# meyerls/PEGASUS

Hardware: AMD Instinct MI355X
Metric: rendered views/sec (RGB+depth+mask) on 2M-Gaussian scene @800x800 (higher is better)
Workload: dtype f32

## Files before the change

### pegasus_amd/csrc/tilebin.hip.h

```cpp
#pragma once
#include <type_traits>

#include "composite.hip.h"
#include "cull.hip.h"
#include "pgr_common.h"

namespace pgr {

constexpr int BIN_CHUNK = 4096;
#ifndef PGR_BIN_THREADS
#define PGR_BIN_THREADS 512
#endif
constexpr int BIN_THREADS = PGR_BIN_THREADS;
constexpr int BIN_LDS_TILES = 16384;

__device__ __forceinline__ uint2 pack_rect(int minx, int miny, int maxx, int maxy) {
    return make_uint2((uint32_t)minx | ((uint32_t)miny << 16), (uint32_t)maxx | ((uint32_t)maxy << 16));
}

struct BinView {
    const uint2* rects;
    const float4* splats;
    uint32_t* tile_count;
    uint32_t* rel;
    uint2* ranges;
    uint32_t* counters;
    uint2* bucket;
    uint32_t* gauss_sorted;
    uint64_t* alt;
    uint32_t* obj_last;
    int32_t n_env;
    const int32_t* tie_index;
    const uint32_t* tie_inv;
    uint2* records;
};


template <int CTRL, int ROW_MASK = 0xF, bool BOUND_CTRL = true>
__device__ __forceinline__ uint32_t dpp_u32(uint32_t v) {
    return (uint32_t)__builtin_amdgcn_update_dpp(0, (int)v, CTRL, ROW_MASK, 0xF, BOUND_CTRL);
}

__device__ __forceinline__ uint32_t wave_inclusive_scan(uint32_t v) {
    v += dpp_u32<0x111>(v);
    v += dpp_u32<0x112>(v);
    v += dpp_u32<0x114>(v);
    v += dpp_u32<0x118>(v);
    v += dpp_u32<0x142, 0xA, false>(v);
    v += dpp_u32<0x143, 0xC, false>(v);
    return v;
}

__device__ __forceinline__ uint32_t wave_inclusive_max(uint32_t v) {
    v = max(v, dpp_u32<0x111>(v));
    v = max(v, dpp_u32<0x112>(v));
    v = max(v, dpp_u32<0x114>(v));
    v = max(v, dpp_u32<0x118>(v));
    v = max(v, dpp_u32<0x142, 0xA, false>(v));
    v = max(v, dpp_u32<0x143, 0xC, false>(v));
    return v;
}

constexpr int BIN_STAGE_WORDS = WAVE * 12 + WAVE;
constexpr int BIN_THREADS_SMALL = 1024;
__host__ __device__ inline size_t bin_lds_bytes(int tiles, int threads) {
    return ((size_t)(tiles < BIN_LDS_TILES ? tiles : BIN_LDS_TILES) + 3) / 4 * 16 + (size_t)(threads / WAVE) * BIN_STAGE_WORDS * 4 + 16;
}

struct BinLayers {
    const int32_t* layer_id;
    int32_t layer_tiles;
    int32_t layer_rows;
    int32_t n_layers;
};
constexpr uint32_t VERDICT_WINDOWS = 62;
constexpr uint32_t VERDICT_REGION_WORDS = 192;

template <bool SCATTER, int THREADS>
__global__ __launch_bounds__(THREADS) void bin_kernel(const BinView* __restrict__ views, int n, int grid_x,
                                                          int tiles, int W, int H, const uint32_t* __restrict__ vis,
                                                          int vis_words, int verdict_groups,
                                                          BinLayers layers = BinLayers{nullptr, 0, 0, 0}) {
    extern __shared__ __attribute__((aligned(16))) uint32_t lds[];
    constexpr int BIN_WAVES = THREADS / WAVE;
    const BinView& bv = views[blockIdx.y];
    if (SCATTER && gload(bv.counters + 1)) return;
    const int chunk = blockIdx.x;
    const int begin = chunk * BIN_CHUNK, end = min(n, begin + BIN_CHUNK);
    const int lane = threadIdx.x & (WAVE - 1), wave = threadIdx.x / WAVE;
    const bool layered = layers.layer_id != nullptr;
    const int hist_words = (min(layered ? layers.layer_tiles : tiles, BIN_LDS_TILES) + 3) / 4 * 4;
    float4* const stage = reinterpret_cast<float4*>(lds + hist_words + wave * BIN_STAGE_WORDS);
    uint32_t* const heads = reinterpret_cast<uint32_t*>(stage + WAVE * 3);
    uint32_t* const ctrl = lds + hist_words + BIN_WAVES * BIN_STAGE_WORDS;
    constexpr int GROUPS = BIN_CHUNK / WAVE;
    static_assert(GROUPS == WAVE, "one visibility bit per lane of a wave");
    int pass_first = 0, pass_last = (tiles - 1) / BIN_LDS_TILES;
    if (layered) {
        if (begin >= end) return;
        pass_first = max(1, min(layers.n_layers + 1, (int)gload(layers.layer_id + begin)));
        pass_last = min(layers.n_layers, (int)gload(layers.layer_id + end - 1));
    }
    for (int lp = pass_first; lp <= pass_last; ++lp) {
        const int lo = layered ? (lp - 1) * layers.layer_tiles : lp * BIN_LDS_TILES;
        const int span = layered ? layers.layer_tiles : min(BIN_LDS_TILES, tiles - lo);
        const int row_off = layered ? (lp - 1) * layers.layer_rows : 0;
        for (int t = threadIdx.x; t < span; t += THREADS)
            lds[t] = SCATTER ? gload(bv.ranges + lo + t).x + gload(bv.rel + (size_t)chunk * tiles + lo + t) : 0u;
        if (wave == 0) {
            const int b = begin + lane * WAVE;
            bool visible = b < end;
            if (visible && vis) visible = (vis[(size_t)(b / WAVE) * vis_words + (blockIdx.y >> 5)] >> (blockIdx.y & 31)) & 1u;
            const uint64_t m = __ballot(visible);
            if (lane == 0) { ctrl[0] = 0u; ctrl[1] = (uint32_t)m; ctrl[2] = (uint32_t)(m >> 32); }
        }
        __syncthreads();
        const uint64_t vis_bits = ((uint64_t)ctrl[2] << 32) | ctrl[1];
        auto take_ticket = [&]() {
            for (;;) {
                uint32_t ticket = 0;
                if (lane == 0) ticket = atomicAdd(&ctrl[0], 1u);
                ticket = (uint32_t)__builtin_amdgcn_readfirstlane((int)ticket);
                if (ticket >= (uint32_t)GROUPS || ((vis_bits >> ticket) & 1ull)) return ticket;
            }
        };
        for (uint32_t ticket = take_ticket(); ticket < (uint32_t)GROUPS; ticket = take_ticket()) {
            const int base = begin + (int)ticket * WAVE;
            bool has_region = base / WAVE < verdict_groups;
            if (layered) {
                const int l0 = gload(layers.layer_id + base), l1 = gload(layers.layer_id + min(base + WAVE, end) - 1);
                if (lp < l0 || lp > l1) continue;
                has_region = has_region && l0 == l1;
            }
            uint32_t* const region = reinterpret_cast<uint32_t*>(bv.records) + (size_t)(base / WAVE) * VERDICT_REGION_WORDS;
            uint64_t* const ballots = reinterpret_cast<uint64_t*>(region + WAVE);
            const int i = base + lane;
            const int ic = i < end ? i : end - 1;
            uint2 r = gload(bv.rects + ic);
            float4 q0 = make_float4(0.f, 0.f, 0.f, 0.f), q1 = q0;
            float depth = 0.0f;
            uint64_t my_ballot = 0;
            if (SCATTER && has_region) {
                depth = __uint_as_float(gload(region + lane));
                if (lane < (int)VERDICT_WINDOWS) my_ballot = gload(ballots + lane);
            } else {
                q0 = gload(bv.splats + (size_t)ic * 3);
                q1 = gload(bv.splats + (size_t)ic * 3 + 1);
                if (SCATTER || has_region) depth = gload(reinterpret_cast<const float*>(bv.splats + (size_t)ic * 3 + 2) + 3);
            }
            if (i >= end) r = make_uint2(0u, 0u);
            const int w = (int)(r.y & 0xffff) - (int)(r.x & 0xffff), h = (int)(r.y >> 16) - (int)(r.x >> 16);
            const uint32_t area = (w > 0 && h > 0) ? (uint32_t)(w * h) : 0u;
            const uint32_t incl = wave_inclusive_scan(area);
            const uint32_t excl = incl - area;
            const uint32_t total = (uint32_t)__builtin_amdgcn_readlane((int)incl, WAVE - 1);
            const bool bits = has_region && total <= VERDICT_WINDOWS * (uint32_t)WAVE;
            if (SCATTER && has_region && !bits) {
                q0 = gload(bv.splats + (size_t)ic * 3);
                q1 = gload(bv.splats + (size_t)ic * 3 + 1);
                depth = gload(reinterpret_cast<const float*>(bv.splats + (size_t)ic * 3 + 2) + 3);
            }
            auto walk = [&](auto from_bits_c, auto write_bits_c) {
                constexpr bool FROM_BITS = decltype(from_bits_c)::value, WRITE_BITS = decltype(write_bits_c)::value;
                float4 s0 = make_float4(0.f, 0.f, 0.f, 0.f), s1 = s0, s2 = s0;
                if (area) {
                    uint32_t flags = 0;
                    if (!FROM_BITS) {
                        const CullSplat cs = make_cull_splat(make_float2(q0.x, q0.y), make_float4(q0.z, q0.w, q1.x, q1.y), q1.z, q1.w);
                        s0 = make_float4(cs.mx, cs.my, cs.A, cs.B);
                        s1 = make_float4(cs.C, cs.rBC, cs.rBA, cs.tau);
                        flags = cs.flags;
                    }
                    s2 = make_float4(__uint_as_float(flags | ((uint32_t)w << 2)), __uint_as_float(r.x), 1.0f / (float)w, depth);
                }
                if (!FROM_BITS) { stage[lane * 3 + 0] = s0; stage[lane * 3 + 1] = s1; }
                stage[lane * 3 + 2] = s2;
                __builtin_amdgcn_wave_barrier();
                if (WRITE_BITS && total) gstore(region + lane, __float_as_uint(depth));
                uint32_t carry_key = 0;
                uint32_t it = 0;
                for (uint32_t c0 = 0; c0 < total; c0 += WAVE, ++it) {
                    uint64_t verdicts = ~0ull;
                    if (FROM_BITS) {
                        const uint32_t vlo = (uint32_t)__builtin_amdgcn_readlane((int)(uint32_t)my_ballot, (int)it);
                        const uint32_t vhi = (uint32_t)__builtin_amdgcn_readlane((int)(uint32_t)(my_ballot >> 32), (int)it);
                        verdicts = ((uint64_t)vhi << 32) | vlo;
                    }
                    heads[lane] = 0u;
                    asm volatile("" ::: "memory");
                    if (area && excl - c0 < (uint32_t)WAVE) heads[excl - c0] = ((excl + 1u) << 6) | (uint32_t)lane;
                    asm volatile("" ::: "memory");
                    uint32_t key = wave_inclusive_max(heads[lane]);
                    asm volatile("" ::: "memory");
                    key = key ? key : carry_key;
                    carry_key = (uint32_t)__builtin_amdgcn_readlane((int)key, WAVE - 1);
                    if (FROM_BITS && verdicts == 0ull) continue;
                    const uint32_t c = c0 + (uint32_t)lane;
                    const int g = (int)(key & 63u);
                    const uint32_t k = c - ((key >> 6) - 1u);
                    const float4 o2 = stage[g * 3 + 2];
                    const uint32_t fw = __float_as_uint(o2.x), rlo = __float_as_uint(o2.y);
                    const int ow = (int)(fw >> 2);
                    int ty = (int)(((float)k + 0.5f) * o2.z);
                    int tx = (int)k - ty * ow;
                    if (tx < 0) { --ty; tx += ow; } else if (tx >= ow) { ++ty; tx -= ow; }
                    const int x = (int)(rlo & 0xffff) + tx, y = (int)(rlo >> 16) + ty;
                    const int t = y * grid_x + x - lo;
                    bool pass = c < total && (unsigned)t < (unsigned)span;
                    if (FROM_BITS) {
                        pass = pass && ((verdicts >> lane) & 1ull);
                    } else if (pass) {
                        const float4 o0 = stage[g * 3 + 0], o1 = stage[g * 3 + 1];
                        CullSplat cs;
                        cs.mx = o0.x; cs.my = o0.y; cs.A = o0.z; cs.B = o0.w;
                        cs.C = o1.x; cs.rBC = o1.y; cs.rBA = o1.z; cs.tau = o1.w; cs.flags = fw & 3u;
                        pass = tile_may_contribute(cs, x, y - row_off, W, H);
                    }
                    if (WRITE_BITS) {
                        const uint64_t m = __ballot(pass);
                        if (lane == 0) gstore(ballots + it, m);
                    }
                    if (pass) {
                        const uint32_t slot = atomicAdd(&lds[t], 1u);
                        if (SCATTER) gstore(bv.bucket + slot, make_uint2(__float_as_uint(o2.w), (uint32_t)(base + g)));
                    }
                }
            };
            if (SCATTER) {
                if (bits) walk(std::true_type{}, std::false_type{}); else walk(std::false_type{}, std::false_type{});
            } else {
                if (bits) walk(std::false_type{}, std::true_type{}); else walk(std::false_type{}, std::false_type{});
            }
        }
        __syncthreads();
        if (!SCATTER) {
            for (int t = threadIdx.x; t < span; t += THREADS) {
                const uint32_t cnt = lds[t];
                gstore(bv.rel + (size_t)chunk * tiles + lo + t, cnt ? gatomic_add(bv.tile_count + lo + t, cnt) : 0u);
            }
            __syncthreads();
        }
    }
}

__global__ void invert_tie_index_kernel(int n, const int32_t* __restrict__ tie_index, uint32_t* __restrict__ tie_inv) {
    const int i = blockIdx.x * blockDim.x + threadIdx.x;
    if (i >= n) return;
    const int k = tie_index[i];
    if ((unsigned)k < (unsigned)n) tie_inv[k] = (uint32_t)i;
}

__global__ __launch_bounds__(1024) void tile_scan_kernel(const BinView* __restrict__ views, int tiles,
                                                         uint32_t max_instances, int grid_x,
                                                         uint32_t* __restrict__ order_state, int skip_empty,
                                                         uint32_t* __restrict__ host_status) {
    __shared__ unsigned long long wave_tot[1024 / WAVE];
    __shared__ unsigned long long carry_s;
    __shared__ uint32_t hist[ORDER_BINS];
    __shared__ uint32_t last_s;
    const BinView& bv = views[blockIdx.x];
    const int lane = threadIdx.x & (WAVE - 1), wid = threadIdx.x / WAVE;
    if (threadIdx.x == 0) carry_s = 0;
    if (threadIdx.x < ORDER_BINS) hist[threadIdx.x] = 0;
    __syncthreads();
    for (int base = 0; base < tiles; base += 1024) {
        const int idx = base + threadIdx.x;
        const unsigned long long v = idx < tiles ? (unsigned long long)bv.tile_count[idx] : 0ull;
        unsigned long long s = v;
#pragma unroll
        for (int d = 1; d < WAVE; d <<= 1) {
            const unsigned long long t = __shfl_up(s, d, WAVE);
            if (lane >= d) s += t;
        }
        if (lane == WAVE - 1) wave_tot[wid] = s;
        __syncthreads();
        unsigned long long wave_prefix = 0;
        for (int w = 0; w < wid; ++w) wave_prefix += wave_tot[w];
        const unsigned long long carry = carry_s;
        const unsigned long long excl = carry + wave_prefix + s - v;
        const unsigned long long cap = max_instances;
        if (idx < tiles) {
            const uint2 r = make_uint2((uint32_t)min(excl, cap), (uint32_t)min(excl + v, cap));
            bv.ranges[idx] = r;
            if (order_state && !(skip_empty && r.y == r.x))
                atomicAdd(&hist[xcd_of_tile(idx, grid_x) * ORDER_CLASSES_USED + coarse_class(r.y - r.x)], ITEMS_PER_TILE);
        }
        __syncthreads();
        if (threadIdx.x == 1023) carry_s = carry + wave_prefix + s;
        __syncthreads();
    }
    if (threadIdx.x == 0) {
        const uint32_t total = (uint32_t)min(carry_s, 0xffffffffull);
        const uint32_t over = carry_s > (unsigned long long)max_instances ? 1u : 0u;
        bv.counters[0] = total;
        bv.counters[1] = over;
        if (host_status) {
            host_status[2 * blockIdx.x] = total;
            host_status[2 * blockIdx.x + 1] = over;
            __threadfence_system();
        }
    }
    if (!order_state) return;
    if (gridDim.x == 1) {
        __syncthreads();
        if (threadIdx.x < NUM_XCD) {
            uint32_t acc = 0;
            for (int c = 0; c < ORDER_CLASSES_USED; ++c) {
                gstore(order_state + threadIdx.x * ORDER_CLASSES_USED + c, acc);
                acc += hist[threadIdx.x * ORDER_CLASSES_USED + c];
            }
        }
        return;
    }
    if (threadIdx.x < ORDER_BINS && hist[threadIdx.x]) gatomic_add(order_state + threadIdx.x, hist[threadIdx.x]);
    __threadfence();
    __syncthreads();
    if (threadIdx.x == 0) last_s = gatomic_add(order_state + ORDER_DONE_WORD, 1u) == gridDim.x - 1u ? 1u : 0u;
    __syncthreads();
    if (!last_s) return;
    __threadfence();
    if (threadIdx.x < NUM_XCD) {
        uint32_t acc = 0;
        for (int c = 0; c < ORDER_CLASSES_USED; ++c) {
            const uint32_t v = gatomic_load(order_state + threadIdx.x * ORDER_CLASSES_USED + c);
            gstore(order_state + threadIdx.x * ORDER_CLASSES_USED + c, acc);
            acc += v;
        }
    }
}

}
```

Measured before the change: 6217.

## Prefetch next bin group loads and batch histogram init/flush memory ops

Unrolls the LDS histogram initialization and the count flush into fixed-trip batches, so all global loads and atomics are issued before any are consumed. In the scatter pass it takes the next ticket early and prefetches that group's rects, depths and first verdict ballots while the current group is walked. Remaining ballot words are loaded only when the group's total area needs them, and the visibility word load is hoisted ahead of the histogram init. This hides global memory latency in the binning kernel, at the cost of more registers (possible occupancy loss) and an explicit waitcnt.

```diff
diff --git a/pegasus_amd/csrc/tilebin.hip.h b/pegasus_amd/csrc/tilebin.hip.h
--- a/pegasus_amd/csrc/tilebin.hip.h
+++ b/pegasus_amd/csrc/tilebin.hip.h
@@ -13,6 +13,7 @@
 #endif
 constexpr int BIN_THREADS = PGR_BIN_THREADS;
 constexpr int BIN_LDS_TILES = 16384;
+constexpr int BIN_FLAT_TRIPS = 8;
 
 __device__ __forceinline__ uint2 pack_rect(int minx, int miny, int maxx, int maxy) {
     return make_uint2((uint32_t)minx | ((uint32_t)miny << 16), (uint32_t)maxx | ((uint32_t)maxy << 16));
@@ -74,6 +75,7 @@
     int32_t n_layers;
 };
 constexpr uint32_t VERDICT_WINDOWS = 62;
+constexpr uint32_t VERDICT_FIRST = 8;
 constexpr uint32_t VERDICT_REGION_WORDS = 192;
 
 template <bool SCATTER, int THREADS>
@@ -88,6 +90,7 @@
     const int chunk = blockIdx.x;
     const int begin = chunk * BIN_CHUNK, end = min(n, begin + BIN_CHUNK);
     const int lane = threadIdx.x & (WAVE - 1), wave = threadIdx.x / WAVE;
+    const uint32_t tid = threadIdx.x;
     const bool layered = layers.layer_id != nullptr;
     const int hist_words = (min(layered ? layers.layer_tiles : tiles, BIN_LDS_TILES) + 3) / 4 * 4;
     float4* const stage = reinterpret_cast<float4*>(lds + hist_words + wave * BIN_STAGE_WORDS);
@@ -105,13 +108,33 @@
         const int lo = layered ? (lp - 1) * layers.layer_tiles : lp * BIN_LDS_TILES;
         const int span = layered ? layers.layer_tiles : min(BIN_LDS_TILES, tiles - lo);
         const int row_off = layered ? (lp - 1) * layers.layer_rows : 0;
-        for (int t = threadIdx.x; t < span; t += THREADS)
-            lds[t] = SCATTER ? gload(bv.ranges + lo + t).x + gload(bv.rel + (size_t)chunk * tiles + lo + t) : 0u;
+        uint32_t vis_word = ~0u;
         if (wave == 0) {
             const int b = begin + lane * WAVE;
-            bool visible = b < end;
-            if (visible && vis) visible = (vis[(size_t)(b / WAVE) * vis_words + (blockIdx.y >> 5)] >> (blockIdx.y & 31)) & 1u;
-            const uint64_t m = __ballot(visible);
+            if (b < end && vis) vis_word = gload(vis + (size_t)(b / WAVE) * vis_words + (blockIdx.y >> 5));
+        }
+        if (SCATTER && span <= BIN_FLAT_TRIPS * THREADS) {
+            const uint2* const range_p = bv.ranges + lo;
+            const uint32_t* const rel_p = bv.rel + (size_t)chunk * tiles + lo;
+            uint32_t start[BIN_FLAT_TRIPS], off[BIN_FLAT_TRIPS];
+#pragma unroll
+            for (int k = 0; k < BIN_FLAT_TRIPS; ++k) {
+                start[k] = 0u; off[k] = 0u;
+                if ((int)tid < span - k * THREADS) {
+                    start[k] = gload(&(range_p + k * THREADS)[tid].x);
+                    off[k] = gload(rel_p + k * THREADS + tid);
+                }
+            }
+#pragma unroll
+            for (int k = 0; k < BIN_FLAT_TRIPS; ++k)
+                if ((int)tid < span - k * THREADS) (lds + k * THREADS)[tid] = start[k] + off[k];
+        } else {
+            for (int t = threadIdx.x; t < span; t += THREADS)
+                lds[t] = SCATTER ? gload(bv.ranges + lo + t).x + gload(bv.rel + (size_t)chunk * tiles + lo + t) : 0u;
+        }
+        if (wave == 0) {
+            const int b = begin + lane * WAVE;
+            const uint64_t m = __ballot(b < end && ((vis_word >> (blockIdx.y & 31)) & 1u));
             if (lane == 0) { ctrl[0] = 0u; ctrl[1] = (uint32_t)m; ctrl[2] = (uint32_t)(m >> 32); }
         }
         __syncthreads();
@@ -124,25 +147,44 @@
                 if (ticket >= (uint32_t)GROUPS || ((vis_bits >> ticket) & 1ull)) return ticket;
             }
         };
-        for (uint32_t ticket = take_ticket(); ticket < (uint32_t)GROUPS; ticket = take_ticket()) {
+        struct GroupLoads { uint2 r; float depth; uint64_t ballot; };
+        auto request = [&](uint32_t ticket) {
+            const int base = begin + (int)ticket * WAVE;
+            const uint32_t* const region = reinterpret_cast<const uint32_t*>(bv.records) + (size_t)(base / WAVE) * VERDICT_REGION_WORDS;
+            GroupLoads g;
+            g.r = gload(bv.rects + min(base + lane, end - 1));
+            g.depth = 0.0f;
+            g.ballot = 0;
+            if (SCATTER && base / WAVE < verdict_groups) {
+                g.depth = __uint_as_float(gload(region + lane));
+                if (lane < (int)VERDICT_FIRST)
+                    g.ballot = gload(reinterpret_cast<const uint64_t*>(region + WAVE) + lane);
+            }
+            return g;
+        };
+        const bool ahead = SCATTER && !layered;
+        uint32_t ticket = take_ticket();
+        GroupLoads pre = ahead && ticket < (uint32_t)GROUPS ? request(ticket) : GroupLoads{make_uint2(0u, 0u), 0.0f, 0};
+        while (ticket < (uint32_t)GROUPS) {
             const int base = begin + (int)ticket * WAVE;
             bool has_region = base / WAVE < verdict_groups;
             if (layered) {
                 const int l0 = gload(layers.layer_id + base), l1 = gload(layers.layer_id + min(base + WAVE, end) - 1);
-                if (lp < l0 || lp > l1) continue;
+                if (lp < l0 || lp > l1) { ticket = take_ticket(); continue; }
                 has_region = has_region && l0 == l1;
             }
             uint32_t* const region = reinterpret_cast<uint32_t*>(bv.records) + (size_t)(base / WAVE) * VERDICT_REGION_WORDS;
             uint64_t* const ballots = reinterpret_cast<uint64_t*>(region + WAVE);
             const int i = base + lane;
             const int ic = i < end ? i : end - 1;
-            uint2 r = gload(bv.rects + ic);
+            const GroupLoads cur = ahead ? pre : request(ticket);
+            uint2 r = cur.r;
             float4 q0 = make_float4(0.f, 0.f, 0.f, 0.f), q1 = q0;
             float depth = 0.0f;
             uint64_t my_ballot = 0;
             if (SCATTER && has_region) {
-                depth = __uint_as_float(gload(region + lane));
-                if (lane < (int)VERDICT_WINDOWS) my_ballot = gload(ballots + lane);
+                depth = cur.depth;
+                my_ballot = cur.ballot;
             } else {
                 q0 = gload(bv.splats + (size_t)ic * 3);
                 q1 = gload(bv.splats + (size_t)ic * 3 + 1);
@@ -155,10 +197,19 @@
             const uint32_t excl = incl - area;
             const uint32_t total = (uint32_t)__builtin_amdgcn_readlane((int)incl, WAVE - 1);
             const bool bits = has_region && total <= VERDICT_WINDOWS * (uint32_t)WAVE;
+            if (SCATTER && bits && total > VERDICT_FIRST * (uint32_t)WAVE && lane >= (int)VERDICT_FIRST &&
+                (uint32_t)lane * WAVE < total)
+                my_ballot = gload(ballots + lane);
             if (SCATTER && has_region && !bits) {
                 q0 = gload(bv.splats + (size_t)ic * 3);
                 q1 = gload(bv.splats + (size_t)ic * 3 + 1);
                 depth = gload(reinterpret_cast<const float*>(bv.splats + (size_t)ic * 3 + 2) + 3);
+            }
+            uint32_t next_ticket = (uint32_t)GROUPS;
+            if (SCATTER) __builtin_amdgcn_s_waitcnt(0x0F70);
+            if (ahead) {
+                next_ticket = take_ticket();
+                if (next_ticket < (uint32_t)GROUPS) pre = request(next_ticket);
             }
             auto walk = [&](auto from_bits_c, auto write_bits_c) {
                 constexpr bool FROM_BITS = decltype(from_bits_c)::value, WRITE_BITS = decltype(write_bits_c)::value;
@@ -231,12 +282,30 @@
             } else {
                 if (bits) walk(std::false_type{}, std::true_type{}); else walk(std::false_type{}, std::false_type{});
             }
+            ticket = ahead ? next_ticket : take_ticket();
         }
         __syncthreads();
         if (!SCATTER) {
-            for (int t = threadIdx.x; t < span; t += THREADS) {
-                const uint32_t cnt = lds[t];
-                gstore(bv.rel + (size_t)chunk * tiles + lo + t, cnt ? gatomic_add(bv.tile_count + lo + t, cnt) : 0u);
+            uint32_t* const count_p = bv.tile_count + lo;
+            uint32_t* const rel_p = bv.rel + (size_t)chunk * tiles + lo;
+            if (span <= BIN_FLAT_TRIPS * THREADS) {
+                uint32_t cnt[BIN_FLAT_TRIPS], off[BIN_FLAT_TRIPS];
+#pragma unroll
+                for (int k = 0; k < BIN_FLAT_TRIPS; ++k)
+                    cnt[k] = (int)tid < span - k * THREADS ? (lds + k * THREADS)[tid] : 0u;
+#pragma unroll
+                for (int k = 0; k < BIN_FLAT_TRIPS; ++k) {
+                    off[k] = 0u;
+                    if (cnt[k]) off[k] = gatomic_add(count_p + k * THREADS + tid, cnt[k]);
+                }
+#pragma unroll
+                for (int k = 0; k < BIN_FLAT_TRIPS; ++k)
+                    if ((int)tid < span - k * THREADS) gstore(rel_p + k * THREADS + tid, off[k]);
+            } else {
+                for (int t = threadIdx.x; t < span; t += THREADS) {
+                    const uint32_t cnt = lds[t];
+                    gstore(rel_p + t, cnt ? gatomic_add(count_p + t, cnt) : 0u);
+                }
             }
             __syncthreads();
         }
```

Result: no change. 6248 (median of 6 runs) (+0.5%).
